# DCGM/pero-pretraining

Hardware: AMD Instinct MI355X
Metric: text-line images/sec (masked-ViT step) (higher is better)
Workload: dtype bf16; 1 GPU; masked pretraining step incl. prepare_batch, 12-layer d=512 h=4 ff=2048 ViT, V=4096, 40x2048 u8 lines (BASELINE.json configs[1]); uint8 images resident in HBM, the PCIe-inclusive rate is `with_h2d`; lines_per_gpu=2048, global_batch=2048, seq_len=256, parallelism=dp1, optimizer=fused Adam (f32 master weights), weight_gradients_on_side_stream=False, head_rows=all, head_backward=masked

## Files before the change

pero_pretraining_amd/csrc/attention_bwd.hip:

```cpp
#include "attention_common.hpp"

template <bool RAGGED = false>
__device__ __forceinline__ void attn_store_tile(const f16v (&acc)[4], unsigned char* stg, bf16raw* out_base, long long ld,
                                                float* colsum, int tid, int wave, int r, int h5, int nrows = 128) {
  __syncthreads();
  const int row_w = wave * 32 + r;
#pragma unroll
  for (int dt = 0; dt < 4; dt++)
#pragma unroll
    for (int g4 = 0; g4 < 4; g4++) {
      uint2 w;
      w.x = pack2bf(acc[dt][4 * g4 + 0], acc[dt][4 * g4 + 1]);
      w.y = pack2bf(acc[dt][4 * g4 + 2], acc[dt][4 * g4 + 3]);
      const int g = dt * 8 + 2 * g4 + h5;
      *(uint2*)(stg + row_w * 256 + ((g ^ (row_w & 31)) << 3)) = w;
    }
  __syncthreads();
  const int ch = tid & 15;
#pragma unroll 2
  for (int i = 0; i < 8; i++) {
    const int row = (tid >> 4) + 16 * i;
    const int x = row & 31;
    uint4 v = *(const uint4*)(stg + row * 256 + ((ch ^ (x >> 1)) << 4));
    if (x & 1) { const unsigned t0 = v.x, t1 = v.y; v.x = v.z; v.y = v.w; v.z = t0; v.w = t1; }
    if (!RAGGED || row < nrows) *(uint4*)(out_base + (long long)row * ld + ch * 8) = v;
  }
  if (colsum) {
    const int lane = tid & 63;
    const int ti = lane & 15, tg = (lane >> 4) & 1;
    const int g = 8 * wave + 4 * tg + (ti & 3);
    const int q0 = 8 * h5 + (ti >> 2);
    const __bf16 one = (__bf16)1.0f;
    const bf8v ones = {one, one, one, one, one, one, one, one};
    f16v cs = {0};
#pragma unroll
    for (int ks = 0; ks < 8; ks++) {
      const int ra = 16 * ks + q0, rb = ra + 4;
      const bf8v frag = lds_tr16_pair(stg + ra * 256 + ((g ^ (ra & 31)) << 3), stg + rb * 256 + ((g ^ (rb & 31)) << 3));
      cs = __builtin_amdgcn_mfma_f32_32x32x16_bf16(ones, frag, cs, 0, 0, 0);
    }
    if (lane < 32) colsum[32 * wave + lane] = cs[0];
  }
}

#define DQ_DEPTH 7
__device__ __forceinline__ constexpr int dq_ninstr(int j) { return (j % 24) < 16 ? 1 : 2; }
__device__ __forceinline__ constexpr int dq_after(int j) {
  int n = 0;
  for (int k = j + 1; k <= j + DQ_DEPTH && k < 48; k++) n += dq_ninstr(k);
  return n;
}
template <bool RAGGED, bool KEYS = false>
__device__ __forceinline__ void attn_bwd_dq_body_p(unsigned char* smem, int lh, int qb, const bf16raw* qkv, const bf16raw* out,
                                                   const bf16raw* dout, const float* lse2, float* dvec, bf16raw* dqkv, float* dbias, int S,
                                                   int nh, float c, float scale, const int* kr = nullptr) {
  const int tid = threadIdx.x, lane = tid & 63, wave = tid >> 6, h5 = lane >> 5, r = lane & 31;
  const int nqb = RAGGED ? (S + 127) >> 7 : S >> 7;
  const int line = lh / nh, head = lh % nh;
  const long long d = (long long)nh * 128, ld = 3 * d;
  const bf16raw* base = qkv + (long long)line * S * ld + head * 128;
  const bf16raw* Kg = base + d;
  const bf16raw* Vg = base + 2 * d;
  const int q = qb * 128 + wave * 32 + r;
  const int qc = RAGGED ? (q < S - 1 ? q : S - 1) : q;
  at_key_range rng = {0, S};
  if constexpr (KEYS) rng = at_load_key_range(kr, line, S);
  const int h0 = KEYS ? rng.k0 >> 6 : 0;

  attn_glds_img<4, RAGGED>(Kg + (long long)h0 * 64 * ld, ld, smem, wave, lane, S - 1 - h0 * 64);
  attn_glds_img<4, RAGGED>(Vg + (long long)h0 * 64 * ld, ld, smem + AT_HALF_BYTES, wave, lane, S - 1 - h0 * 64);

  bf8v qf[8], gf[8];
  float dsum = 0.f;
  const long long dix = ((long long)line * S + qc) * nh + head;
  {
    const bf16raw* qrow = base + (long long)qc * ld + 8 * h5;
    const bf16raw* grow = dout + ((long long)line * S + qc) * d + head * 128 + 8 * h5;
#pragma unroll
    for (int ks = 0; ks < 8; ks++) {
      qf[ks] = *(const bf8v*)(qrow + 16 * ks);
      gf[ks] = *(const bf8v*)(grow + 16 * ks);
    }
    if (out) {
      const bf16raw* orow = out + ((long long)line * S + qc) * d + head * 128 + 8 * h5;
#pragma unroll
      for (int ks = 0; ks < 8; ks++) {
        const bf8v of = *(const bf8v*)(orow + 16 * ks);
#pragma unroll
        for (int e = 0; e < 8; e++) dsum += (float)gf[ks][e] * (float)of[e];
      }
      dsum += __shfl_xor(dsum, 32, 64);
      if (h5 == 0 && (!RAGGED || q < S)) dvec[dix] = dsum;
    } else {
      dsum = dvec[dix];
    }
  }
  const float lq = lse2[(long long)lh * S + qc];

  const unsigned s0 = at_lds_addr(smem);
  unsigned ra[8], ta[4], tb[4];
  {
    const int f = img_f(r);
#pragma unroll
    for (int ks = 0; ks < 8; ks++) ra[ks] = (unsigned)(r * 256 + (((2 * ks + h5) ^ f) << 4));
    const int i = lane & 15, g1 = (lane >> 4) & 1;
    const int row = 4 * h5 + (i >> 2);
#pragma unroll
    for (int dt = 0; dt < 4; dt++) {
      const int ch = 4 * dt + 2 * g1 + ((i & 3) >> 1);
      ta[dt] = (unsigned)(row * 256 + ((ch ^ img_f(row)) << 4) + 8 * (i & 1));
      tb[dt] = (unsigned)((row + 8) * 256 + ((ch ^ img_f(row + 8)) << 4) + 8 * (i & 1));
    }
  }

  f16v dq[4];
#pragma unroll
  for (int t = 0; t < 4; t++) dq[t] = (f16v){0};
  const int nhalf = KEYS ? ((rng.k1 + 63) >> 6) - h0 : RAGGED ? (S + 63) >> 6 : S >> 6;
  for (int hk = 0; hk < nhalf; hk++) {
    asm volatile("s_waitcnt vmcnt(0)" ::: "memory");
    __syncthreads();
    const unsigned stage = s0 + (hk & 1) * 2 * AT_HALF_BYTES;
    if (hk + 1 < nhalf) {
      unsigned char* nb = smem + ((hk + 1) & 1) * 2 * AT_HALF_BYTES;
      attn_glds_img<4, RAGGED>(Kg + (long long)(h0 + hk + 1) * 64 * ld, ld, nb, wave, lane, S - 1 - (h0 + hk + 1) * 64);
      attn_glds_img<4, RAGGED>(Vg + (long long)(h0 + hk + 1) * 64 * ld, ld, nb + AT_HALF_BYTES, wave, lane, S - 1 - (h0 + hk + 1) * 64);
    }
    bf8v fr[8];
    f16v s, dp;
    bf8v dsf[2];
    auto issue = [&](auto jc) __attribute__((always_inline)) {
      constexpr int j = decltype(jc)::value;
      constexpr int t = j / 24, qd = j % 24;
      if constexpr (qd < 16) {
        constexpr int ks = qd >> 1, isv = qd & 1;
        at_rd128<isv * AT_HALF_BYTES + t * 8192>(fr[j & 7], ra[ks], stage);
      } else {
        constexpr int sub = (qd - 16) >> 2, dt = (qd - 16) & 3;
        at_rdtr<t * 8192 + sub * 4096, t * 8192 + sub * 4096>(fr[j & 7], ta[dt], tb[dt], stage);
      }
    };
    at_static_for<0, DQ_DEPTH>(issue);
    AT_PRIO(1);
    at_static_for<0, 48>([&](auto jc) __attribute__((always_inline)) {
      constexpr int j = decltype(jc)::value;
      constexpr int qd = j % 24;
      if constexpr (j + DQ_DEPTH < 48) issue(std::integral_constant<int, j + DQ_DEPTH>{});
      if constexpr (qd == 16) {
        AT_PRIO(0);
#pragma unroll
        for (int e = 0; e < 16; e++) {
          const float p = __builtin_amdgcn_exp2f(fmaf(s[e], c, -lq));
          s[e] = p * (dp[e] - dsum) * scale;
        }
        if constexpr (KEYS) {
          if (hk == 0 || hk == nhalf - 1 || qb == nqb - 1) {
            constexpr int t = j / 24;
            const int lo = rng.k0 - (h0 + hk) * 64 - t * 32 - 4 * h5;
            const int hi = q < S ? rng.k1 - (h0 + hk) * 64 - t * 32 - 4 * h5 : lo;
#pragma unroll
            for (int e = 0; e < 16; e++) {
              const int k = 8 * (e >> 2) + (e & 3);
              s[e] = (k >= lo && k < hi) ? s[e] : 0.f;
            }
          }
        } else if (RAGGED && (hk == nhalf - 1 || qb == nqb - 1)) {
          constexpr int t = j / 24;
          const int lim = q < S ? S - hk * 64 - t * 32 - 4 * h5 : 0;
#pragma unroll
          for (int e = 0; e < 16; e++) s[e] = (8 * (e >> 2) + (e & 3) < lim) ? s[e] : 0.f;
        }
        dsf[0] = pack8(s, 0);
        dsf[1] = pack8(s, 1);
        AT_PRIO(1);
      }
      at_wait_lgkm<dq_after(j)>(fr[j & 7]);
      if constexpr (qd < 16) {
        constexpr int ks = qd >> 1;
        if constexpr (qd == 0) s = __builtin_amdgcn_mfma_f32_32x32x16_bf16(fr[j & 7], qf[0], (f16v){0}, 0, 0, 0);
        else if constexpr (qd == 1) dp = __builtin_amdgcn_mfma_f32_32x32x16_bf16(fr[j & 7], gf[0], (f16v){0}, 0, 0, 0);
        else if constexpr ((qd & 1) == 0) s = __builtin_amdgcn_mfma_f32_32x32x16_bf16(fr[j & 7], qf[ks], s, 0, 0, 0);
        else dp = __builtin_amdgcn_mfma_f32_32x32x16_bf16(fr[j & 7], gf[ks], dp, 0, 0, 0);
      } else {
        constexpr int sub = (qd - 16) >> 2, dt = (qd - 16) & 3;
        dq[dt] = __builtin_amdgcn_mfma_f32_32x32x16_bf16(fr[j & 7], dsf[sub], dq[dt], 0, 0, 0);
      }
    });
    AT_PRIO(0);
  }
  attn_store_tile<RAGGED>(dq, smem, dqkv + ((long long)line * S + qb * 128) * ld + head * 128, ld,
                          dbias ? dbias + ((long long)lh * nqb + qb) * 128 : nullptr, tid, wave, r, h5, S - qb * 128);
}
template <bool RAGGED>
__global__ __launch_bounds__(256, 2) void attn_bwd_dq_k(const bf16raw* qkv, const bf16raw* out, const bf16raw* dout, const float* lse2,
                                                        float* dvec, bf16raw* dqkv, float* dbias, int S, int nh, float c, float scale) {
  extern __shared__ __attribute__((aligned(16))) unsigned char smem[];
  const int nqb = RAGGED ? (S + 127) >> 7 : S >> 7;
  int lh, qb;
  attn_block_map(blockIdx.x, nqb, gridDim.x / nqb, lh, qb);
  attn_bwd_dq_body_p<RAGGED>(smem, lh, qb, qkv, out, dout, lse2, dvec, dqkv, dbias, S, nh, c, scale);
}

#ifndef DKV_POOL
#define DKV_POOL 6
#endif
#define DKV_TD (DKV_POOL - 1)
#define DKV_RDEPTH (DKV_POOL - 2)
template <bool RAGGED, bool KEYS = false>
__device__ __forceinline__ void attn_bwd_dkv2_body_p(unsigned char* smem, int lh, int kb, long long nwg, const bf16raw* qkv, const bf16raw* dout,
                                                     const float* lse2, const float* dvec, bf16raw* dqkv, float* dbias, int S, int nh, float c,
                                                     float scale, const int* kr = nullptr) {
  unsigned char* vimg = smem + 4 * AT_SUB_BYTES;
  float* lds_ld = (float*)(smem + 4 * AT_SUB_BYTES + AT_TILE_BYTES);
  const int tid = threadIdx.x, lane = tid & 63, wave = tid >> 6, h5 = lane >> 5, r = lane & 31;
  const int nkb = RAGGED ? (S + 127) >> 7 : S >> 7;
  const int line = lh / nh, head = lh % nh;
  const long long d = (long long)nh * 128, ld = 3 * d;
  const bf16raw* base = qkv + (long long)line * S * ld + head * 128;
  const bf16raw* Gg = dout + (long long)line * S * d + head * 128;
  const int key = kb * 128 + wave * 32 + r;
  const int kc = RAGGED ? (key < S - 1 ? key : S - 1) : key;
  const float* stat = tid < 32 ? lse2 + (long long)lh * S + tid : dvec + ((long long)line * S + (tid & 31)) * nh + head;
  const long long stat_step = tid < 32 ? 32 : 32LL * nh;
  int stat_tail = 0;
  if constexpr (RAGGED) {
    const int qs = (((S + 31) >> 5) - 1) * 32 + (tid & 31);
    stat_tail = qs < S ? 0 : (S - 1 - qs) * (tid < 32 ? 1 : nh);
  }

  if constexpr (RAGGED) { if (tid < 64) lds_ld[tid] = stat[S <= 32 ? stat_tail : 0]; }
  else if (tid < 64) lds_ld[tid] = stat[0];
  attn_glds_img<8, RAGGED>(base + 2 * d + (long long)kb * 128 * ld, ld, vimg, wave, lane, S - 1 - kb * 128);
  attn_glds_img<2, RAGGED>(base, ld, smem, wave, lane, S - 1);
  attn_glds_img<2, RAGGED>(Gg, d, smem + AT_SUB_BYTES, wave, lane, S - 1);

  bf8v kf[8];
  {
    const bf16raw* krow = base + d + (long long)kc * ld + 8 * h5;
#pragma unroll
    for (int ks = 0; ks < 8; ks++) kf[ks] = *(const bf8v*)(krow + 16 * ks);
  }
  const unsigned s0 = at_lds_addr(smem);
  const unsigned vbase = s0 + 4 * AT_SUB_BYTES + __builtin_amdgcn_readfirstlane(wave) * 8192;
  unsigned ra[8], ta[4], tb[4];
  {
    const int f = img_f(r);
#pragma unroll
    for (int ks = 0; ks < 8; ks++) ra[ks] = (unsigned)(r * 256 + (((2 * ks + h5) ^ f) << 4));
    const int i = lane & 15, g1 = (lane >> 4) & 1;
    const int row = 4 * h5 + (i >> 2);
#pragma unroll
    for (int dt = 0; dt < 4; dt++) {
      const int ch = 4 * dt + 2 * g1 + ((i & 3) >> 1);
      ta[dt] = (unsigned)(row * 256 + ((ch ^ img_f(row)) << 4) + 8 * (i & 1));
      tb[dt] = (unsigned)((row + 8) * 256 + ((ch ^ img_f(row + 8)) << 4) + 8 * (i & 1));
    }
  }
  f16v dv[4], dk[4];
#pragma unroll
  for (int t = 0; t < 4; t++) { dv[t] = (f16v){0}; dk[t] = (f16v){0}; }
  at_key_range rng = {0, S};
  if constexpr (KEYS) rng = at_load_key_range(kr, line, S);
  const bool dead_tile = KEYS && (kb * 128 >= rng.k1 || kb * 128 + 128 <= rng.k0);
  const int nsub = dead_tile ? 0 : RAGGED ? (S + 31) >> 5 : S >> 5;
  for (int sq = 0; sq < nsub; sq++) {
    asm volatile("s_waitcnt vmcnt(0)" ::: "memory");
    __syncthreads();
    const unsigned stage = s0 + (sq & 1) * 2 * AT_SUB_BYTES;
    const float* lds_l = lds_ld + (sq & 1) * 64;
    const float* lds_d = lds_l + 32;
    float nstat = 0.f;
    if (sq + 1 < nsub) {
      if constexpr (RAGGED) { if (tid < 64) nstat = stat[(sq + 1) * stat_step + (sq + 2 == nsub ? stat_tail : 0)]; }
      else if (tid < 64) nstat = stat[(sq + 1) * stat_step];
      unsigned char* nb = smem + ((sq + 1) & 1) * 2 * AT_SUB_BYTES;
      attn_glds_img<2, RAGGED>(base + (long long)(sq + 1) * 32 * ld, ld, nb, wave, lane, S - 1 - (sq + 1) * 32);
      attn_glds_img<2, RAGGED>(Gg + (long long)(sq + 1) * 32 * d, d, nb + AT_SUB_BYTES, wave, lane, S - 1 - (sq + 1) * 32);
    }
    bf8v fr[DKV_POOL];
    f16v s, dp;
    auto issue_r = [&](auto jc) __attribute__((always_inline)) {
      constexpr int j = decltype(jc)::value;
      constexpr int ks = j / 3, kind = j % 3;
      if constexpr (kind == 0) at_rd128<0>(fr[j % DKV_POOL], ra[ks], stage);
      else if constexpr (kind == 1) at_rd128<AT_SUB_BYTES>(fr[j % DKV_POOL], ra[ks], stage);
      else at_rd128<0>(fr[j % DKV_POOL], ra[ks], vbase);
    };
    at_static_for<0, DKV_RDEPTH>(issue_r);
    AT_PRIO(1);
    at_static_for<0, 24>([&](auto jc) __attribute__((always_inline)) {
      constexpr int j = decltype(jc)::value;
      constexpr int ks = j / 3, kind = j % 3;
      if constexpr (j + DKV_RDEPTH < 24) issue_r(std::integral_constant<int, j + DKV_RDEPTH>{});
      constexpr int after = (24 - 1 - j) < DKV_RDEPTH ? (24 - 1 - j) : DKV_RDEPTH;
      if constexpr (kind == 0) {
        at_wait_lgkm<after>(fr[j % DKV_POOL]);
        if constexpr (ks == 0) s = __builtin_amdgcn_mfma_f32_32x32x16_bf16(fr[j % DKV_POOL], kf[0], (f16v){0}, 0, 0, 0);
        else s = __builtin_amdgcn_mfma_f32_32x32x16_bf16(fr[j % DKV_POOL], kf[ks], s, 0, 0, 0);
      } else if constexpr (kind == 2) {
        at_wait_lgkm<after>(fr[j % DKV_POOL]);
        asm volatile("" : "+v"(fr[(j - 1) % DKV_POOL]));
        if constexpr (ks == 0) dp = __builtin_amdgcn_mfma_f32_32x32x16_bf16(fr[(j - 1) % DKV_POOL], fr[j % DKV_POOL], (f16v){0}, 0, 0, 0);
        else dp = __builtin_amdgcn_mfma_f32_32x32x16_bf16(fr[(j - 1) % DKV_POOL], fr[j % DKV_POOL], dp, 0, 0, 0);
      }
    });
    AT_PRIO(0);
    auto issue_t = [&](auto mc) __attribute__((always_inline)) {
      constexpr int m = decltype(mc)::value;
      constexpr int sub = m >> 3, dt = (m >> 1) & 3, kind = m & 1;
      constexpr int off = sub * 4096 + (kind == 0 ? AT_SUB_BYTES : 0);
      at_rdtr<off, off>(fr[m % DKV_POOL], ta[dt], tb[dt], stage);
    };
    f4v l4[4], d4[4];
    const unsigned stb = s0 + 4 * AT_SUB_BYTES + AT_TILE_BYTES + (sq & 1) * 256, sto = 16 * h5;
    auto issue_s = [&](auto gc) __attribute__((always_inline)) {
      constexpr int g = decltype(gc)::value;
      at_rd128<32 * g>(l4[g], sto, stb);
      at_rd128<128 + 32 * g>(d4[g], sto, stb);
    };
    issue_s(std::integral_constant<int, 0>{});
    issue_s(std::integral_constant<int, 1>{});
    bf8v pf[2], dsf[2];
    at_static_for<0, 4>([&](auto gc) __attribute__((always_inline)) {
      constexpr int g4 = decltype(gc)::value;
      constexpr int after = g4 == 0 ? 2 : g4 == 1 ? 6 : g4 == 2 ? 10 : (DKV_TD >= 6 ? 8 : 4);
      at_wait_lgkm2<after>(l4[g4], d4[g4]);
#pragma unroll
      for (int e = 0; e < 4; e++) {
        float p = __builtin_amdgcn_exp2f(fmaf(s[4 * g4 + e], c, -l4[g4][e]));
        if constexpr (RAGGED) p = (sq * 32 + 8 * g4 + 4 * h5 + e < S) ? p : 0.f;
        s[4 * g4 + e] = p;
        dp[4 * g4 + e] = p * (dp[4 * g4 + e] - d4[g4][e]) * scale;
      }
      if constexpr (g4 == 1) { pf[0] = pack8(s, 0); dsf[0] = pack8(dp, 0); }
      if constexpr (g4 == 3) { pf[1] = pack8(s, 1); dsf[1] = pack8(dp, 1); }
      if constexpr (g4 + 2 < 4) issue_s(std::integral_constant<int, g4 + 2>{});
      if constexpr (2 * g4 < DKV_TD) issue_t(std::integral_constant<int, 2 * g4>{});
      if constexpr (2 * g4 + 1 < DKV_TD) issue_t(std::integral_constant<int, 2 * g4 + 1>{});
    });
    AT_PRIO(1);
    at_static_for<0, 16>([&](auto mc) __attribute__((always_inline)) {
      constexpr int m = decltype(mc)::value;
      constexpr int sub = m >> 3, dt = (m >> 1) & 3, kind = m & 1;
      if constexpr (m + DKV_TD < 16) issue_t(std::integral_constant<int, m + DKV_TD>{});
      constexpr int after = 2 * ((16 - 1 - m) < DKV_TD ? (16 - 1 - m) : DKV_TD);
      at_wait_lgkm<after>(fr[m % DKV_POOL]);
      if constexpr (kind == 0) dv[dt] = __builtin_amdgcn_mfma_f32_32x32x16_bf16(fr[m % DKV_POOL], pf[sub], dv[dt], 0, 0, 0);
      else dk[dt] = __builtin_amdgcn_mfma_f32_32x32x16_bf16(fr[m % DKV_POOL], dsf[sub], dk[dt], 0, 0, 0);
    });
    AT_PRIO(0);
    if (sq + 1 < nsub && tid < 64) lds_ld[((sq + 1) & 1) * 64 + tid] = nstat;
  }
  if constexpr (KEYS) asm volatile("s_waitcnt vmcnt(0)" ::: "memory");
  if constexpr (RAGGED) {
    const bool live = KEYS ? (key >= rng.k0 && key < rng.k1) : key < S;
#pragma unroll
    for (int t = 0; t < 4; t++)
#pragma unroll
      for (int e = 0; e < 16; e++) { dk[t][e] = live ? dk[t][e] : 0.f; dv[t][e] = live ? dv[t][e] : 0.f; }
  }
  bf16raw* tile_o = dqkv + ((long long)line * S + kb * 128) * ld + d + head * 128;
  attn_store_tile<RAGGED>(dk, smem, tile_o, ld, dbias ? dbias + (nwg + (long long)lh * nkb + kb) * 128 : nullptr, tid, wave, r, h5, S - kb * 128);
  attn_store_tile<RAGGED>(dv, smem, tile_o + d, ld, dbias ? dbias + (2 * nwg + (long long)lh * nkb + kb) * 128 : nullptr, tid, wave, r, h5, S - kb * 128);
}
template <bool RAGGED>
__global__ __launch_bounds__(256, 2) void attn_bwd_dkv2_k(const bf16raw* qkv, const bf16raw* dout, const float* lse2, const float* dvec,
                                                          bf16raw* dqkv, float* dbias, int S, int nh, float c, float scale) {
  extern __shared__ __attribute__((aligned(16))) unsigned char smem[];
  const int nkb = RAGGED ? (S + 127) >> 7 : S >> 7;
  int lh, kb;
  attn_block_map(blockIdx.x, nkb, gridDim.x / nkb, lh, kb);
  attn_bwd_dkv2_body_p<RAGGED>(smem, lh, kb, gridDim.x, qkv, dout, lse2, dvec, dqkv, dbias, S, nh, c, scale);
}
__device__ __forceinline__ void attn_pair_map(int nb, int order, int& lh, int& blk) {
  attn_block_map(blockIdx.x, 2 * nb, gridDim.x / (2 * nb), lh, blk);
  {
    const int nlh = gridDim.x / (2 * nb);
    if (order && (nlh & 7) == 0) {
      const int xcd = blockIdx.x & 7, u = blockIdx.x >> 3;
      if (order == 1) blk = (blk + nb) % (2 * nb);
      else {
        const int CH = order % 100, v = order / 100, per = CH * 2 * nb;
        if (CH > 0 && (nlh >> 3) % CH == 0) {
          const int cch = u / per, i = u % per, first = i / (CH * nb), j = i % (CH * nb);
          const int role_dkv = (v & 1) ? first : 1 - first;
          const int un = (v & 2) ? j % CH : j / nb, bl = (v & 2) ? j / CH : j % nb;
          lh = (cch * CH + un) * 8 + xcd;
          blk = (role_dkv ? nb : 0) + bl;
        }
      }
    }
  }
}
template <bool RAGGED>
__global__ __launch_bounds__(256, 2) void attn_bwd_pair_k(const bf16raw* qkv, const bf16raw* dout, const float* lse2, float* dvec,
                                                          bf16raw* dqkv, float* dbias, int S, int nh, float c, float scale, int order) {
  extern __shared__ __attribute__((aligned(16))) unsigned char smem[];
  const int nb = RAGGED ? (S + 127) >> 7 : S >> 7;
  int lh, blk;
  attn_pair_map(nb, order, lh, blk);
  if (blk < nb) attn_bwd_dq_body_p<RAGGED>(smem, lh, blk, qkv, nullptr, dout, lse2, dvec, dqkv, dbias, S, nh, c, scale);
  else attn_bwd_dkv2_body_p<RAGGED>(smem, lh, blk - nb, (long long)(gridDim.x >> 1), qkv, dout, lse2, dvec, dqkv, dbias, S, nh, c, scale);
}
__global__ __launch_bounds__(256, 2) void attn_bwd_dq_keys_k(const bf16raw* qkv, const int* kr, const bf16raw* out, const bf16raw* dout, const float* lse2,
                                                             float* dvec, bf16raw* dqkv, float* dbias, int S, int nh, float c, float scale) {
  extern __shared__ __attribute__((aligned(16))) unsigned char smem[];
  const int nqb = (S + 127) >> 7;
  int lh, qb;
  attn_block_map(blockIdx.x, nqb, gridDim.x / nqb, lh, qb);
  attn_bwd_dq_body_p<true, true>(smem, lh, qb, qkv, out, dout, lse2, dvec, dqkv, dbias, S, nh, c, scale, kr);
}
__global__ __launch_bounds__(256, 2) void attn_bwd_dkv2_keys_k(const bf16raw* qkv, const int* kr, const bf16raw* dout, const float* lse2, const float* dvec,
                                                               bf16raw* dqkv, float* dbias, int S, int nh, float c, float scale) {
  extern __shared__ __attribute__((aligned(16))) unsigned char smem[];
  const int nkb = (S + 127) >> 7;
  int lh, kb;
  attn_block_map(blockIdx.x, nkb, gridDim.x / nkb, lh, kb);
  attn_bwd_dkv2_body_p<true, true>(smem, lh, kb, gridDim.x, qkv, dout, lse2, dvec, dqkv, dbias, S, nh, c, scale, kr);
}
__global__ __launch_bounds__(256, 2) void attn_bwd_pair_keys_k(const bf16raw* qkv, const int* kr, const bf16raw* dout, const float* lse2, float* dvec,
                                                               bf16raw* dqkv, float* dbias, int S, int nh, float c, float scale, int order) {
  extern __shared__ __attribute__((aligned(16))) unsigned char smem[];
  const int nb = (S + 127) >> 7;
  int lh, blk;
  attn_pair_map(nb, order, lh, blk);
  if (blk < nb) attn_bwd_dq_body_p<true, true>(smem, lh, blk, qkv, nullptr, dout, lse2, dvec, dqkv, dbias, S, nh, c, scale, kr);
  else attn_bwd_dkv2_body_p<true, true>(smem, lh, blk - nb, (long long)(gridDim.x >> 1), qkv, dout, lse2, dvec, dqkv, dbias, S, nh, c, scale, kr);
}

constexpr int AT_PAIR_LDS = AT_DKV2_LDS > 2 * AT_TILE_BYTES ? AT_DKV2_LDS : 2 * AT_TILE_BYTES;

static int attn_bwd_run(const char* who, const void* qkv, const int* key_ranges , const void* out, const void* dout, const float* lse,
                        float* dvec, void* dqkv, float* dbias, float* work, int64_t N, int64_t S, int64_t num_heads, int64_t head_dim, int dtype,
                        hipStream_t st) {
  PERO_REQUIRE(qkv && dout && lse && dvec && dqkv, "%s: null pointer", who);
  PERO_REQUIRE(dtype == PERO_BF16 && (head_dim == 64 || head_dim == 128) && S > 0 && N > 0 && num_heads > 0,
               "%s: fused kernel needs bf16, head_dim 64 or 128, S > 0 (got hd=%lld S=%lld)", who, (long long)head_dim, (long long)S);
  PERO_REQUIRE(aligned16(qkv) && (!out || aligned16(out)) && aligned16(dout) && aligned16(dqkv), "%s: 16-byte alignment", who);
  PERO_REQUIRE(!dbias || work, "%s: dbias needs the partial-sum workspace", who);
  if (head_dim == 64) {
    attn64_bwd_launch(qkv, key_ranges, out, dout, lse, dvec, dqkv, dbias, work, N, S, num_heads, st);
    PERO_CHECK_LAUNCH(who);
    return PERO_OK;
  }
  PERO_LDS_ATTR(attn_bwd_dq_k<false>, 2 * AT_TILE_BYTES);
  PERO_LDS_ATTR(attn_bwd_dq_k<true>, 2 * AT_TILE_BYTES);
  PERO_LDS_ATTR(attn_bwd_dq_keys_k, 2 * AT_TILE_BYTES);
  PERO_LDS_ATTR(attn_bwd_dkv2_k<false>, AT_DKV2_LDS);
  PERO_LDS_ATTR(attn_bwd_dkv2_k<true>, AT_DKV2_LDS);
  PERO_LDS_ATTR(attn_bwd_dkv2_keys_k, AT_DKV2_LDS);
  PERO_LDS_ATTR(attn_bwd_pair_k<false>, AT_PAIR_LDS);
  PERO_LDS_ATTR(attn_bwd_pair_k<true>, AT_PAIR_LDS);
  PERO_LDS_ATTR(attn_bwd_pair_keys_k, AT_PAIR_LDS);
  const float scale = (float)(1.0 / sqrt((double)head_dim));
  const float c = (float)(1.4426950408889634 / sqrt((double)head_dim));
  const int64_t nb = (S + 127) / 128;
  const bool ragged = S % 128 != 0;
  const dim3 grid((unsigned)(N * num_heads * nb)), block(256);
  const bf16raw *q_ = (const bf16raw*)qkv, *o_ = (const bf16raw*)out, *g_ = (const bf16raw*)dout;
  bf16raw* dq_ = (bf16raw*)dqkv;
  float* const part = dbias ? work : nullptr;
  const int s_ = (int)S, nh_ = (int)num_heads;
  if (!out && g_opt.attn_bwd_pair) {
    const dim3 grid2(2 * grid.x);
    if (key_ranges) hipLaunchKernelGGL(attn_bwd_pair_keys_k, grid2, block, AT_PAIR_LDS, st, q_, key_ranges, g_, lse, dvec, dq_, part, s_, nh_, c, scale, g_opt.attn_order);
    else hipLaunchKernelGGL((ragged ? attn_bwd_pair_k<true> : attn_bwd_pair_k<false>), grid2, block, AT_PAIR_LDS, st, q_, g_, lse, dvec, dq_, part, s_, nh_, c, scale, g_opt.attn_order);
  } else if (key_ranges) {
    hipLaunchKernelGGL(attn_bwd_dq_keys_k, grid, block, 2 * AT_TILE_BYTES, st, q_, key_ranges, o_, g_, lse, dvec, dq_, part, s_, nh_, c, scale);
    hipLaunchKernelGGL(attn_bwd_dkv2_keys_k, grid, block, AT_DKV2_LDS, st, q_, key_ranges, g_, lse, dvec, dq_, part, s_, nh_, c, scale);
  } else {
    hipLaunchKernelGGL((ragged ? attn_bwd_dq_k<true> : attn_bwd_dq_k<false>), grid, block, 2 * AT_TILE_BYTES, st, q_, o_, g_, lse, dvec, dq_, part, s_, nh_, c, scale);
    hipLaunchKernelGGL((ragged ? attn_bwd_dkv2_k<true> : attn_bwd_dkv2_k<false>), grid, block, AT_DKV2_LDS, st, q_, g_, lse, dvec, dq_, part, s_, nh_, c, scale);
  }
  if (dbias) attn_bias_reduce_launch<128>(work, dbias, N, num_heads, nb, st);
  PERO_CHECK_LAUNCH(who);
  return PERO_OK;
}

extern "C" int pero_attention_bwd(const void* qkv, const void* out, const void* dout, const float* lse, float* dvec, void* dqkv,
                                  float* dbias, float* work, int64_t N, int64_t S, int64_t num_heads, int64_t head_dim, int dtype,
                                  void* stream) {
  return attn_bwd_run("pero_attention_bwd", qkv, nullptr, out, dout, lse, dvec, dqkv, dbias, work, N, S, num_heads, head_dim, dtype, (hipStream_t)stream);
}

extern "C" int pero_attention_bwd_keys(const void* qkv, const int* key_ranges, const void* out, const void* dout, const float* lse, float* dvec, void* dqkv,
                                       float* dbias, float* work, int64_t N, int64_t S, int64_t num_heads, int64_t head_dim, int dtype, void* stream) {
  PERO_REQUIRE(key_ranges, "pero_attention_bwd_keys: null pointer");
  return attn_bwd_run("pero_attention_bwd_keys", qkv, key_ranges, out, dout, lse, dvec, dqkv, dbias, work, N, S, num_heads, head_dim, dtype, (hipStream_t)stream);
}
```

pero_pretraining_amd/csrc/attention_common.hpp:

```cpp
#pragma once
#include "common.hpp"
#include "options.hpp"
#include <type_traits>

#define AT_TILE_BYTES (128 * 128 * 2)
#define AT_HALF_BYTES 16384
#define AT_SUB_BYTES 8192
#define AT_DKV2_LDS (4 * AT_SUB_BYTES + 128 * 128 * 2 + 512)
#define AT_PRIO(n_) __builtin_amdgcn_s_setprio(n_)
typedef short s8v __attribute__((ext_vector_type(8)));

struct at_no_limit { __device__ constexpr at_no_limit(int = 0) {} };
struct at_row_limit { int last; __device__ constexpr at_row_limit(int l) : last(l) {} };
template <bool RAGGED> using at_limit = std::conditional_t<RAGGED, at_row_limit, at_no_limit>;
template <bool VIMG, bool RAGGED = false>
__device__ __forceinline__ void attn_glds_tile(const bf16raw* g, long long ld, unsigned char* lds, int wave, int lane, at_limit<RAGGED> lim = {}) {
#pragma unroll
  for (int i = 0; i < 8; i++) {
    const int p = wave + 4 * i;
    const int row = 4 * p + (lane >> 4), slot = lane & 15;
    const int chunk = VIMG ? ((((slot >> 2) ^ (row & 3)) << 2) | (slot & 3)) : (slot ^ (row & 15));
    int srow = row;
    if constexpr (RAGGED) srow = row < lim.last ? row : lim.last;
    __builtin_amdgcn_global_load_lds((const __attribute__((address_space(1))) void*)(g + (long long)srow * ld + chunk * 8),
                                     (__attribute__((address_space(3))) void*)(lds + p * 1024), 16, 0, 0);
  }
}
__device__ __forceinline__ int img_f(int row) { return ((row & 3) << 2) | ((row >> 2) & 3); }
template <int NP, bool RAGGED = false>
__device__ __forceinline__ void attn_glds_img(const bf16raw* g, long long ld, unsigned char* lds, int wave, int lane, at_limit<RAGGED> lim = {}) {
#pragma unroll
  for (int i = 0; i < NP; i++) {
    const int p = wave + 4 * i;
    const int row = 4 * p + (lane >> 4), slot = lane & 15;
    const int chunk = slot ^ img_f(row);
    int srow = row;
    if constexpr (RAGGED) srow = row < lim.last ? row : lim.last;
    __builtin_amdgcn_global_load_lds((const __attribute__((address_space(1))) void*)(g + (long long)srow * ld + chunk * 8),
                                     (__attribute__((address_space(3))) void*)(lds + p * 1024), 16, 0, 0);
  }
}

__device__ __forceinline__ bf8v attn_k_frag(const unsigned char* kimg, int key, int ks, int h5) {
  const int chunk = 2 * ks + h5;
  return *(const bf8v*)(kimg + key * 256 + ((chunk ^ (key & 15)) << 4));
}
__device__ __forceinline__ bf8v attn_vT_frag(const unsigned char* vimg, int kb, int dt, int lane) {
  const int i = lane & 15, g1 = (lane >> 4) & 1, h5 = lane >> 5;
  const int key = kb + 4 * h5 + (i >> 2);
  const unsigned char* a = vimg + key * 256 + ((dt ^ (key & 3)) << 6) + g1 * 32 + (i & 3) * 8;
  s4v lo = __builtin_amdgcn_ds_read_tr16_b64_v4i16(LDS_PTR(s4v, a));
  s4v hi = __builtin_amdgcn_ds_read_tr16_b64_v4i16(LDS_PTR(s4v, a + 8 * 256));
  s8v v = {lo[0], lo[1], lo[2], lo[3], hi[0], hi[1], hi[2], hi[3]};
  return __builtin_bit_cast(bf8v, v);
}
__device__ __forceinline__ bf8v pack8(const f16v& a, int s) {
  typedef unsigned u4v __attribute__((ext_vector_type(4)));
  u4v u = {pack2bf(a[8 * s + 0], a[8 * s + 1]), pack2bf(a[8 * s + 2], a[8 * s + 3]), pack2bf(a[8 * s + 4], a[8 * s + 5]),
           pack2bf(a[8 * s + 6], a[8 * s + 7])};
  return __builtin_bit_cast(bf8v, u);
}

__device__ __forceinline__ bf8v img_row_frag(const unsigned char* img, int row, int ks, int h5) {
  return *(const bf8v*)(img + row * 256 + (((2 * ks + h5) ^ img_f(row)) << 4));
}
__device__ __forceinline__ bf8v img_tr_frag(const unsigned char* img, int rb, int dt, int lane) {
  const int i = lane & 15, g1 = (lane >> 4) & 1, h5 = lane >> 5;
  const int row = rb + 4 * h5 + (i >> 2);
  const int ch = 4 * dt + 2 * g1 + ((i & 3) >> 1);
  const unsigned char* a = img + row * 256 + ((ch ^ img_f(row)) << 4) + 8 * (i & 1);
  const unsigned char* b = img + (row + 8) * 256 + ((ch ^ img_f(row + 8)) << 4) + 8 * (i & 1);
  s4v lo = __builtin_amdgcn_ds_read_tr16_b64_v4i16(LDS_PTR(s4v, a));
  s4v hi = __builtin_amdgcn_ds_read_tr16_b64_v4i16(LDS_PTR(s4v, b));
  s8v v = {lo[0], lo[1], lo[2], lo[3], hi[0], hi[1], hi[2], hi[3]};
  return __builtin_bit_cast(bf8v, v);
}

struct at_key_range { int k0, k1; };
__device__ __forceinline__ at_key_range at_load_key_range(const int* kr, int line, int S) {
  int k0 = kr[2 * line], k1 = kr[2 * line + 1];
  k0 = k0 < 0 ? 0 : (k0 > S - 1 ? S - 1 : k0);
  k1 = k1 < k0 + 1 ? k0 + 1 : (k1 > S ? S : k1);
  return {k0, k1};
}

__device__ __forceinline__ void attn_block_map(int bid, int nblk, int nlh, int& lh, int& blk) {
  if ((nlh & 7) == 0) {
    const int xcd = bid & 7, u = bid >> 3;
    lh = (u / nblk) * 8 + xcd;
    blk = u % nblk;
  } else {
    lh = bid / nblk;
    blk = bid % nblk;
  }
}

template <int I, int N, typename F>
__device__ __forceinline__ void at_static_for(F&& f) {
  if constexpr (I < N) {
    f(std::integral_constant<int, I>{});
    at_static_for<I + 1, N>(f);
  }
}
typedef int at_i2v __attribute__((ext_vector_type(2)));
typedef unsigned at_u2v __attribute__((ext_vector_type(2)));
typedef unsigned at_u4v __attribute__((ext_vector_type(4)));
typedef int at_i4v __attribute__((ext_vector_type(4)));
__device__ __forceinline__ unsigned at_lds_addr(const void* p) { return (unsigned)(unsigned long long)LDS_PTR(const unsigned char, p); }
template <int OFF, typename T>
__device__ __forceinline__ void at_rd128(T& d, unsigned lane_off, unsigned base) {
  static_assert(sizeof(T) == 16, "ds_read_b128");
  unsigned a;
  asm volatile("v_add_u32 %1, %3, %2\n\tds_read_b128 %0, %1 offset:%4" : "=v"(d), "=&v"(a) : "v"(lane_off), "s"(base), "i"(OFF) : "memory");
}
template <int OFFA, int OFFB>
__device__ __forceinline__ void at_rdtr(bf8v& d, unsigned off_a, unsigned off_b, unsigned base) {
  at_i2v lo, hi;
  unsigned a, b;
  asm volatile("v_add_u32 %2, %6, %4\n\tv_add_u32 %3, %6, %5\n\tds_read_b64_tr_b16 %0, %2 offset:%7\n\tds_read_b64_tr_b16 %1, %3 offset:%8"
               : "=&v"(lo), "=&v"(hi), "=&v"(a), "=&v"(b) : "v"(off_a), "v"(off_b), "s"(base), "i"(OFFA), "i"(OFFB) : "memory");
  d = __builtin_bit_cast(bf8v, __builtin_shufflevector(lo, hi, 0, 1, 2, 3));
}
template <int OFF, typename T>
__device__ __forceinline__ void at_rd128a(T& d, unsigned addr) {
  static_assert(sizeof(T) == 16, "ds_read_b128");
  asm volatile("ds_read_b128 %0, %1 offset:%2" : "=v"(d) : "v"(addr), "i"(OFF) : "memory");
}
template <int OFFA, int OFFB>
__device__ __forceinline__ void at_rdtra(bf8v& d, unsigned addr_a, unsigned addr_b) {
  at_i2v lo, hi;
  asm volatile("ds_read_b64_tr_b16 %0, %2 offset:%4\n\tds_read_b64_tr_b16 %1, %3 offset:%5"
               : "=&v"(lo), "=&v"(hi) : "v"(addr_a), "v"(addr_b), "i"(OFFA), "i"(OFFB) : "memory");
  d = __builtin_bit_cast(bf8v, __builtin_shufflevector(lo, hi, 0, 1, 2, 3));
}
template <int OFF, int KX, typename T>
__device__ __forceinline__ void at_rd128x(T& d, unsigned lane_off, unsigned base) {
  static_assert(sizeof(T) == 16, "ds_read_b128");
  unsigned a;
  asm volatile("v_xor_b32 %1, %4, %2\n\tv_add_u32 %1, %3, %1\n\tds_read_b128 %0, %1 offset:%5" : "=v"(d), "=&v"(a) : "v"(lane_off), "s"(base), "i"(KX), "i"(OFF) : "memory");
}
template <int OFFA, int OFFB, int KX>
__device__ __forceinline__ void at_rdtrx(bf8v& d, unsigned off_a, unsigned off_b, unsigned base) {
  at_i2v lo, hi;
  unsigned a, b;
  asm volatile("v_xor_b32 %2, %7, %4\n\tv_xor_b32 %3, %7, %5\n\tv_add_u32 %2, %6, %2\n\tv_add_u32 %3, %6, %3\n\tds_read_b64_tr_b16 %0, %2 offset:%8\n\tds_read_b64_tr_b16 %1, %3 offset:%9"
               : "=&v"(lo), "=&v"(hi), "=&v"(a), "=&v"(b) : "v"(off_a), "v"(off_b), "s"(base), "i"(KX), "i"(OFFA), "i"(OFFB) : "memory");
  d = __builtin_bit_cast(bf8v, __builtin_shufflevector(lo, hi, 0, 1, 2, 3));
}
template <int N, typename T>
__device__ __forceinline__ void at_wait_lgkm(T& f) {
  static_assert(N >= 0 && N <= 15, "lgkmcnt is a 4-bit counter");
  asm volatile("s_waitcnt lgkmcnt(%1)" : "+v"(f) : "i"(N) : "memory");
}
template <int N, typename T>
__device__ __forceinline__ void at_wait_lgkm2(T& f, T& g) {
  static_assert(N >= 0 && N <= 15, "lgkmcnt is a 4-bit counter");
  asm volatile("s_waitcnt lgkmcnt(%2)" : "+v"(f), "+v"(g) : "i"(N) : "memory");
}

template <int IMM, typename T>
__device__ __forceinline__ void at_gload16(T& d, const void* sbase, unsigned voff) {
  static_assert(sizeof(T) == 16 && IMM >= 0 && IMM < 4096, "global_load_dwordx4");
  asm volatile("s_nop 4\n\tglobal_load_dwordx4 %0, %1, %2 offset:%3" : "=v"(d) : "v"(voff), "s"(sbase), "i"(IMM) : "memory");
}
template <int IMM, typename T>
__device__ __forceinline__ void at_gstore16(const T& v, void* sbase, unsigned voff) {
  static_assert(sizeof(T) == 16 && IMM >= 0 && IMM < 4096, "global_store_dwordx4");
  asm volatile("s_nop 4\n\tglobal_store_dwordx4 %0, %1, %2 offset:%3\n\ts_nop 2" :: "v"(voff), "v"(v), "s"(sbase), "i"(IMM) : "memory");
}
__device__ __forceinline__ void at_gstore4(float v, void* sbase, unsigned voff) {
  asm volatile("s_nop 4\n\tglobal_store_dword %0, %1, %2\n\ts_nop 2" :: "v"(voff), "v"(v), "s"(sbase) : "memory");
}
__device__ __forceinline__ void at_barrier() {
  __builtin_amdgcn_sched_barrier(0);
  asm volatile("s_barrier" ::: "memory");
  __builtin_amdgcn_sched_barrier(0);
}
template <typename T>
__device__ __forceinline__ void at_ds_write8(unsigned addr, const T& v) {
  static_assert(sizeof(T) == 8, "ds_write_b64");
  asm volatile("ds_write_b64 %0, %1" :: "v"(addr), "v"(v) : "memory");
}
template <typename T>
__device__ __forceinline__ void at_ds_read16(T& d, unsigned addr) {
  static_assert(sizeof(T) == 16, "ds_read_b128");
  asm volatile("ds_read_b128 %0, %1" : "=v"(d) : "v"(addr) : "memory");
}
template <int N>
__device__ __forceinline__ void at_wait_lgkm_plain() {
  asm volatile("s_waitcnt lgkmcnt(%0)" :: "i"(N) : "memory");
}

template <int HD>
__global__ __launch_bounds__(HD) void attn_bias_reduce_k(const float* partial, float* dbias, int nlines, int nh, int nblk) {
  const int c = threadIdx.x, head = blockIdx.x, which = blockIdx.y;
  const long long nwg = (long long)nlines * nh * nblk;
  const float* p = partial + (long long)which * nwg * HD;
  const int per_head = nlines * nblk;
  const int chunk = (per_head + gridDim.z - 1) / gridDim.z;
  const int i0 = blockIdx.z * chunk, i1 = i0 + chunk < per_head ? i0 + chunk : per_head;
  float s[8] = {0.f, 0.f, 0.f, 0.f, 0.f, 0.f, 0.f, 0.f};
  auto at = [&](int i) -> float { return p[(((long long)(i / nblk) * nh + head) * nblk + i % nblk) * HD + c]; };
  int i = i0;
  for (; i + 8 <= i1; i += 8) {
#pragma unroll
    for (int k = 0; k < 8; k++) s[k] += at(i + k);
  }
  for (; i < i1; i++) s[0] += at(i);
  if (i0 < i1) atomicAdd(dbias + (long long)which * nh * HD + head * HD + c, ((s[0] + s[1]) + (s[2] + s[3])) + ((s[4] + s[5]) + (s[6] + s[7])));
}
template <int HD>
static inline void attn_bias_reduce_launch(const float* partial, float* dbias, int64_t N, int64_t num_heads, int64_t nb, hipStream_t st) {
  const unsigned slices = (N * nb >= 4096) ? 128 : (N * nb >= 1024) ? 64 : 16;
  hipLaunchKernelGGL(attn_bias_reduce_k<HD>, dim3((unsigned)num_heads, 3, slices), dim3(HD), 0, st, partial, dbias, (int)N, (int)num_heads, (int)nb);
}

__attribute__((visibility("hidden"))) void attn64_fwd_launch(const void* qkv, const int* kr, void* out, float* lse, int64_t N, int64_t S, int64_t num_heads, hipStream_t st);
__attribute__((visibility("hidden"))) void attn64_bwd_launch(const void* qkv, const int* kr, const void* out, const void* dout, const float* lse, float* dvec, void* dqkv,
                                                             float* dbias, float* work, int64_t N, int64_t S, int64_t num_heads, hipStream_t st);
```

Before: 14260 lines/s.

## Triple-buffer dK/dV query stages and load softmax stats via registers with DPP broadcast

New measurement: 14170 lines/s. No clear change (-0.6%).

```diff
diff --git a/pero_pretraining_amd/csrc/attention_bwd.hip b/pero_pretraining_amd/csrc/attention_bwd.hip
--- a/pero_pretraining_amd/csrc/attention_bwd.hip
+++ b/pero_pretraining_amd/csrc/attention_bwd.hip
@@ -210,8 +210,7 @@
 __device__ __forceinline__ void attn_bwd_dkv2_body_p(unsigned char* smem, int lh, int kb, long long nwg, const bf16raw* qkv, const bf16raw* dout,
                                                      const float* lse2, const float* dvec, bf16raw* dqkv, float* dbias, int S, int nh, float c,
                                                      float scale, const int* kr = nullptr) {
-  unsigned char* vimg = smem + 4 * AT_SUB_BYTES;
-  float* lds_ld = (float*)(smem + 4 * AT_SUB_BYTES + AT_TILE_BYTES);
+  unsigned char* vimg = smem + 6 * AT_SUB_BYTES;
   const int tid = threadIdx.x, lane = tid & 63, wave = tid >> 6, h5 = lane >> 5, r = lane & 31;
   const int nkb = RAGGED ? (S + 127) >> 7 : S >> 7;
   const int line = lh / nh, head = lh % nh;
@@ -220,28 +219,43 @@
   const bf16raw* Gg = dout + (long long)line * S * d + head * 128;
   const int key = kb * 128 + wave * 32 + r;
   const int kc = RAGGED ? (key < S - 1 ? key : S - 1) : key;
-  const float* stat = tid < 32 ? lse2 + (long long)lh * S + tid : dvec + ((long long)line * S + (tid & 31)) * nh + head;
-  const long long stat_step = tid < 32 ? 32 : 32LL * nh;
-  int stat_tail = 0;
-  if constexpr (RAGGED) {
-    const int qs = (((S + 31) >> 5) - 1) * 32 + (tid & 31);
-    stat_tail = qs < S ? 0 : (S - 1 - qs) * (tid < 32 ? 1 : nh);
-  }
-
-  if constexpr (RAGGED) { if (tid < 64) lds_ld[tid] = stat[S <= 32 ? stat_tail : 0]; }
-  else if (tid < 64) lds_ld[tid] = stat[0];
+  at_key_range rng = {0, S};
+  if constexpr (KEYS) rng = at_load_key_range(kr, line, S);
+  const bool dead_tile = KEYS && (kb * 128 >= rng.k1 || kb * 128 + 128 <= rng.k0);
+  const int nstage = RAGGED ? (S + 31) >> 5 : S >> 5;
+  const int nsub = dead_tile ? 0 : nstage;
+  const unsigned qrow4 = 4u * (8 * ((lane & 15) >> 2) + (lane & 3) + 4 * h5);
+  const float* stat_l = lse2 + (long long)lh * S;
+  const float* stat_d = dvec + (long long)line * S * nh + head;
+  float ln, dn;
+  auto load_stat = [&](int st) __attribute__((always_inline)) {
+    const unsigned lim4 = (RAGGED && st == nstage - 1) ? 4u * (unsigned)(S - 1 - st * 32) : 124u;
+    unsigned ol, od;
+    asm volatile("v_min_u32 %0, %3, %2\n\tv_mul_lo_u32 %1, %0, %4" : "=&v"(ol), "=&v"(od) : "v"(qrow4), "s"(lim4), "s"(nh));
+    at_gload4(ln, stat_l + (long long)st * 32, ol);
+    at_gload4(dn, stat_d + (long long)st * 32 * nh, od);
+  };
+  auto load_stage = [&](int st, int slot) __attribute__((always_inline)) {
+    unsigned char* nb = smem + slot * 2 * AT_SUB_BYTES;
+    attn_glds_img<2, RAGGED>(base + (long long)st * 32 * ld, ld, nb, wave, lane, S - 1 - st * 32);
+    attn_glds_img<2, RAGGED>(Gg + (long long)st * 32 * d, d, nb + AT_SUB_BYTES, wave, lane, S - 1 - st * 32);
+  };
+
+  load_stat(0);
   attn_glds_img<8, RAGGED>(base + 2 * d + (long long)kb * 128 * ld, ld, vimg, wave, lane, S - 1 - kb * 128);
-  attn_glds_img<2, RAGGED>(base, ld, smem, wave, lane, S - 1);
-  attn_glds_img<2, RAGGED>(Gg, d, smem + AT_SUB_BYTES, wave, lane, S - 1);
-
+  load_stage(0, 0);
   bf8v kf[8];
   {
-    const bf16raw* krow = base + d + (long long)kc * ld + 8 * h5;
-#pragma unroll
-    for (int ks = 0; ks < 8; ks++) kf[ks] = *(const bf8v*)(krow + 16 * ks);
-  }
+    const bf16raw* ktile = base + d + (long long)kb * 128 * ld;
+    const unsigned kvoff = (unsigned)(kc - kb * 128) * (unsigned)(2 * ld) + 16 * h5;
+    at_static_for<0, 8>([&](auto kc_) __attribute__((always_inline)) {
+      constexpr int ks = decltype(kc_)::value;
+      at_gload16<32 * ks>(kf[ks], ktile, kvoff);
+    });
+  }
+  if (nsub > 1) load_stage(1, 1);
   const unsigned s0 = at_lds_addr(smem);
-  const unsigned vbase = s0 + 4 * AT_SUB_BYTES + __builtin_amdgcn_readfirstlane(wave) * 8192;
+  const unsigned vbase = s0 + 6 * AT_SUB_BYTES + __builtin_amdgcn_readfirstlane(wave) * 8192;
   unsigned ra[8], ta[4], tb[4];
   {
     const int f = img_f(r);
@@ -259,24 +273,18 @@
   f16v dv[4], dk[4];
 #pragma unroll
   for (int t = 0; t < 4; t++) { dv[t] = (f16v){0}; dk[t] = (f16v){0}; }
-  at_key_range rng = {0, S};
-  if constexpr (KEYS) rng = at_load_key_range(kr, line, S);
-  const bool dead_tile = KEYS && (kb * 128 >= rng.k1 || kb * 128 + 128 <= rng.k0);
-  const int nsub = dead_tile ? 0 : RAGGED ? (S + 31) >> 5 : S >> 5;
+  int slot = 0;
   for (int sq = 0; sq < nsub; sq++) {
-    asm volatile("s_waitcnt vmcnt(0)" ::: "memory");
-    __syncthreads();
-    const unsigned stage = s0 + (sq & 1) * 2 * AT_SUB_BYTES;
-    const float* lds_l = lds_ld + (sq & 1) * 64;
-    const float* lds_d = lds_l + 32;
-    float nstat = 0.f;
-    if (sq + 1 < nsub) {
-      if constexpr (RAGGED) { if (tid < 64) nstat = stat[(sq + 1) * stat_step + (sq + 2 == nsub ? stat_tail : 0)]; }
-      else if (tid < 64) nstat = stat[(sq + 1) * stat_step];
-      unsigned char* nb = smem + ((sq + 1) & 1) * 2 * AT_SUB_BYTES;
-      attn_glds_img<2, RAGGED>(base + (long long)(sq + 1) * 32 * ld, ld, nb, wave, lane, S - 1 - (sq + 1) * 32);
-      attn_glds_img<2, RAGGED>(Gg + (long long)(sq + 1) * 32 * d, d, nb + AT_SUB_BYTES, wave, lane, S - 1 - (sq + 1) * 32);
-    }
+    asm volatile("s_waitcnt vmcnt(4)\n\ts_cmp_lg_u32 %10, 0\n\ts_cbranch_scc1 .Lat_dkv_w%=\n\ts_waitcnt vmcnt(0)\n.Lat_dkv_w%=:"
+                 : "+v"(ln), "+v"(dn), "+v"(kf[0]), "+v"(kf[1]), "+v"(kf[2]), "+v"(kf[3]), "+v"(kf[4]), "+v"(kf[5]), "+v"(kf[6]), "+v"(kf[7])
+                 : "s"(__builtin_amdgcn_readfirstlane(nsub - 1 - sq)) : "memory", "scc");
+    at_barrier();
+    const unsigned stage = s0 + slot * 2 * AT_SUB_BYTES;
+    float lc, dc;
+    asm volatile("v_mov_b32 %0, %2\n\tv_mov_b32 %1, %3" : "=&v"(lc), "=&v"(dc) : "v"(ln), "v"(dn));
+    load_stat(sq + 1 < nstage ? sq + 1 : nstage - 1);
+    if (sq + 2 < nsub) load_stage(sq + 2, slot == 0 ? 2 : slot - 1);
+    slot = slot == 2 ? 0 : slot + 1;
     bf8v fr[DKV_POOL];
     f16v s, dp;
     auto issue_r = [&](auto jc) __attribute__((always_inline)) {
@@ -311,30 +319,18 @@
       constexpr int off = sub * 4096 + (kind == 0 ? AT_SUB_BYTES : 0);
       at_rdtr<off, off>(fr[m % DKV_POOL], ta[dt], tb[dt], stage);
     };
-    f4v l4[4], d4[4];
-    const unsigned stb = s0 + 4 * AT_SUB_BYTES + AT_TILE_BYTES + (sq & 1) * 256, sto = 16 * h5;
-    auto issue_s = [&](auto gc) __attribute__((always_inline)) {
-      constexpr int g = decltype(gc)::value;
-      at_rd128<32 * g>(l4[g], sto, stb);
-      at_rd128<128 + 32 * g>(d4[g], sto, stb);
-    };
-    issue_s(std::integral_constant<int, 0>{});
-    issue_s(std::integral_constant<int, 1>{});
     bf8v pf[2], dsf[2];
     at_static_for<0, 4>([&](auto gc) __attribute__((always_inline)) {
       constexpr int g4 = decltype(gc)::value;
-      constexpr int after = g4 == 0 ? 2 : g4 == 1 ? 6 : g4 == 2 ? 10 : (DKV_TD >= 6 ? 8 : 4);
-      at_wait_lgkm2<after>(l4[g4], d4[g4]);
-#pragma unroll
-      for (int e = 0; e < 4; e++) {
-        float p = __builtin_amdgcn_exp2f(fmaf(s[4 * g4 + e], c, -l4[g4][e]));
+      at_static_for<0, 4>([&](auto ec) __attribute__((always_inline)) {
+        constexpr int e = decltype(ec)::value;
+        float p = __builtin_amdgcn_exp2f(fmaf(s[4 * g4 + e], c, -at_row_bcast<4 * g4 + e>(lc)));
         if constexpr (RAGGED) p = (sq * 32 + 8 * g4 + 4 * h5 + e < S) ? p : 0.f;
         s[4 * g4 + e] = p;
-        dp[4 * g4 + e] = p * (dp[4 * g4 + e] - d4[g4][e]) * scale;
-      }
+        dp[4 * g4 + e] = p * (dp[4 * g4 + e] - at_row_bcast<4 * g4 + e>(dc)) * scale;
+      });
       if constexpr (g4 == 1) { pf[0] = pack8(s, 0); dsf[0] = pack8(dp, 0); }
       if constexpr (g4 == 3) { pf[1] = pack8(s, 1); dsf[1] = pack8(dp, 1); }
-      if constexpr (g4 + 2 < 4) issue_s(std::integral_constant<int, g4 + 2>{});
       if constexpr (2 * g4 < DKV_TD) issue_t(std::integral_constant<int, 2 * g4>{});
       if constexpr (2 * g4 + 1 < DKV_TD) issue_t(std::integral_constant<int, 2 * g4 + 1>{});
     });
@@ -349,9 +345,8 @@
       else dk[dt] = __builtin_amdgcn_mfma_f32_32x32x16_bf16(fr[m % DKV_POOL], dsf[sub], dk[dt], 0, 0, 0);
     });
     AT_PRIO(0);
-    if (sq + 1 < nsub && tid < 64) lds_ld[((sq + 1) & 1) * 64 + tid] = nstat;
-  }
-  if constexpr (KEYS) asm volatile("s_waitcnt vmcnt(0)" ::: "memory");
+  }
+  asm volatile("s_waitcnt vmcnt(0)" : "+v"(ln), "+v"(dn), "+v"(kf[0]), "+v"(kf[1]), "+v"(kf[2]), "+v"(kf[3]), "+v"(kf[4]), "+v"(kf[5]), "+v"(kf[6]), "+v"(kf[7]) :: "memory");
   if constexpr (RAGGED) {
     const bool live = KEYS ? (key >= rng.k0 && key < rng.k1) : key < S;
 #pragma unroll
diff --git a/pero_pretraining_amd/csrc/attention_common.hpp b/pero_pretraining_amd/csrc/attention_common.hpp
--- a/pero_pretraining_amd/csrc/attention_common.hpp
+++ b/pero_pretraining_amd/csrc/attention_common.hpp
@@ -6,7 +6,7 @@
 #define AT_TILE_BYTES (128 * 128 * 2)
 #define AT_HALF_BYTES 16384
 #define AT_SUB_BYTES 8192
-#define AT_DKV2_LDS (4 * AT_SUB_BYTES + 128 * 128 * 2 + 512)
+#define AT_DKV2_LDS (6 * AT_SUB_BYTES + AT_TILE_BYTES)
 #define AT_PRIO(n_) __builtin_amdgcn_s_setprio(n_)
 typedef short s8v __attribute__((ext_vector_type(8)));
 
@@ -158,11 +158,16 @@
   asm volatile("s_waitcnt lgkmcnt(%2)" : "+v"(f), "+v"(g) : "i"(N) : "memory");
 }
 
+template <int IMM, int BYTES, typename T>
+__device__ __forceinline__ void at_gload(T& d, const void* sbase, unsigned voff) {
+  static_assert(sizeof(T) == BYTES && (BYTES == 4 || BYTES == 16) && IMM >= 0 && IMM < 4096, "global_load_dword / global_load_dwordx4");
+  asm volatile("s_nop 4\n\t.if %4 == 16\n\tglobal_load_dwordx4 %0, %1, %2 offset:%3\n\t.else\n\tglobal_load_dword %0, %1, %2 offset:%3\n\t.endif"
+               : "=v"(d) : "v"(voff), "s"(sbase), "i"(IMM), "i"(BYTES) : "memory");
+}
 template <int IMM, typename T>
-__device__ __forceinline__ void at_gload16(T& d, const void* sbase, unsigned voff) {
-  static_assert(sizeof(T) == 16 && IMM >= 0 && IMM < 4096, "global_load_dwordx4");
-  asm volatile("s_nop 4\n\tglobal_load_dwordx4 %0, %1, %2 offset:%3" : "=v"(d) : "v"(voff), "s"(sbase), "i"(IMM) : "memory");
-}
+__device__ __forceinline__ void at_gload16(T& d, const void* sbase, unsigned voff) { at_gload<IMM, 16>(d, sbase, voff); }
+template <typename T>
+__device__ __forceinline__ void at_gload4(T& d, const void* sbase, unsigned voff) { at_gload<0, 4>(d, sbase, voff); }
 template <int IMM, typename T>
 __device__ __forceinline__ void at_gstore16(const T& v, void* sbase, unsigned voff) {
   static_assert(sizeof(T) == 16 && IMM >= 0 && IMM < 4096, "global_store_dwordx4");
@@ -185,6 +190,11 @@
 __device__ __forceinline__ void at_ds_read16(T& d, unsigned addr) {
   static_assert(sizeof(T) == 16, "ds_read_b128");
   asm volatile("ds_read_b128 %0, %1" : "=v"(d) : "v"(addr) : "memory");
+}
+template <int N>
+__device__ __forceinline__ float at_row_bcast(float v) {
+  static_assert(N >= 0 && N < 16, "row_newbcast");
+  return __builtin_bit_cast(float, __builtin_amdgcn_update_dpp(0, __builtin_bit_cast(int, v), 0x150 + N, 0xf, 0xf, true));
 }
 template <int N>
 __device__ __forceinline__ void at_wait_lgkm_plain() {
```
